# channable/alfred-margaret

Hardware: AMD Instinct MI355X
Metric: GiB/s haystack bytes scanned (match-emitting runLower, 100k-needle automaton) (higher is better)
Workload: dtype u8

## Files before the change

### alfred-margaret_amd/api.py

```python
import ctypes as C
import os

import numpy as np

from . import build as _build

CASE_SENSITIVE = 0
IGNORE_CASE = 1

AM_OK = 0
AM_ERR_INVALID, AM_ERR_NO_DEVICE, AM_ERR_HIP, AM_ERR_OOM, AM_ERR_UNSUPPORTED = -1, -2, -3, -4, -5


class AmError(RuntimeError):
    def __init__(self, code, msg):
        super().__init__("libam error %d: %s" % (code, msg))
        self.code = code


class _Match:
    __slots__ = ()

    def __repr__(self):
        return "am.MATCH"
# ... 1944 lines not shown
SF_MODES = ("count", "emit", "any", "ids")


def decode_sf_variant(word):
    word = int(word)
    if not word & 1:
        return None
    return {"ic": bool(word & 2), "mode": SF_MODES[(word >> 2) & 3], "ilp": (word >> 4) & 3, "lw": (word >> 16) & 255, "short": bool(word & 64), "dbg": bool(word & 128),
            "light": bool(word & 256), "children": bool(word & 512)}


def sf_last_variant():
    return decode_sf_variant(libam().am_debug_sf_last_variant())


def bounds_report():
    f, l, u = C.c_uint64(0), C.c_uint32(0), C.c_uint32(0)
    check(libam().am_debug_bounds_report(C.byref(f), C.byref(l), C.byref(u)))
    return int(f.value), int(l.value), int(u.value)


def image_version():
    return int(libam().am_image_version())


def lower_code_point(cp):
    return int(libam().am_lower_code_point(cp))


def unlower_code_point(cp):
# ... 49 lines not shown
```

### alfred-margaret_amd/csrc/am_abi.cpp

```cpp
#include "am_host.h"

#include <condition_variable>
#include <deque>
#include <sys/mman.h>

using namespace am;
using namespace am::dev;
using namespace am::host;

static_assert(sizeof(am_match) == sizeof(Record), "am_match must mirror the device record");
static_assert(offsetof(am_match, end_pos) == offsetof(Record, end_pos) && offsetof(am_match, haystack) == offsetof(Record, haystack) &&
                  offsetof(am_match, state) == offsetof(Record, state), "am_match layout");


static thread_local std::string g_err;
namespace am { int abi_fail(int code, const std::string& msg) { g_err = msg; return code; } }

namespace am {
namespace host {

Runtime g_rt;

int ensure_runtime()
{
// ... 208 lines not shown
{
    Orphans& o = orphans();
    std::lock_guard<std::mutex> lk(o.mu);
    for (int d = 0; d < kMaxDev; d++) {
        if (oneshot[d]) { o.batches[d].push_back(oneshot[d]); oneshot[d] = nullptr; }
        if (own[d]) { o.streams[d].push_back(own[d]); own[d] = nullptr; }
    }
    if (pin || pin_res) { o.pins.push_back(Orphans::Pins{pin, pin_cap, pin_res, pin_res_cap}); pin = pin_res = nullptr; }
    for (int k = 0; k < 2; k++) if (pin_ev[k] && pin_ev_dev >= 0) { o.events[pin_ev_dev].push_back(pin_ev[k]); pin_ev[k] = nullptr; }
}
}


uint64_t am::host::next_image_generation() { static std::atomic<uint64_t> g{0}; return g.fetch_add(1, std::memory_order_relaxed) + 1u; }

int am::host::prepare(const am_automaton* ca, int case_mode, const Flavor** out)
{
    if (!ca) return fail(AM_ERR_INVALID, "null automaton");
    if (case_mode != AM_CASE_SENSITIVE && case_mode != AM_IGNORE_CASE) return fail(AM_ERR_INVALID, "bad case_mode");
    am_automaton* a = const_cast<am_automaton*>(ca);
    std::lock_guard<std::mutex> lk(a->mu);
    Flavor& f = a->fl[case_mode];
    if (!f.ready) {
        if (!a->has_ref) return fail(AM_ERR_UNSUPPORTED, "this handle was attached to an image of the other case mode");
        AM_TRY(ensure_runtime());
        ON_DEVICE(a->dev);
        std::vector<uint8_t> img; std::string err;
        if (case_mode == AM_CASE_SENSITIVE && !a->cs_image.empty()) img.swap(a->cs_image);
        else if (case_mode == AM_IGNORE_CASE && a->ic_pending.valid()) {
            am_automaton::Flat fl = a->ic_pending.get();
            if (fl.rc != 0) return fail(AM_ERR_INVALID, fl.err);
            img.swap(fl.img);
        }
        else {
            RefArrays ref{a->transitions.data(), a->transitions.size(), a->offsets.data(), a->offsets.size() - 1, a->root_ascii.data(), a->values_len.data()};
            if (flatten(ref, case_mode, img, err, a->lower.get()) != 0) return fail(AM_ERR_INVALID, err);
        }
        void* d = nullptr;
        hipError_t e = hipMalloc(&d, img.size());
        if (e != hipSuccess) return fail(AM_ERR_OOM, std::string("hipMalloc(image): ") + hipGetErrorString(e));
        e = hipMemcpy(d, img.data(), img.size(), hipMemcpyHostToDevice);
        if (e != hipSuccess) { (void)hipFree(d); return fail(AM_ERR_HIP, std::string("hipMemcpy(image): ") + hipGetErrorString(e)); }
        std::memcpy(&f.h, img.data(), sizeof(ImageHeader));
        f.d_image = d; f.bytes = img.size(); f.generation = next_image_generation(); f.ready = true;
    }
    *out = &f;
    return AM_OK;
}

extern "C" const char* am_last_error(void) { return g_err.c_str(); }

extern "C" int am_automaton_create_ex(const uint64_t* transitions, size_t n_transitions, const uint32_t* offsets, size_t n_states,
                                      const uint64_t* root_ascii, const uint32_t* values_len,
                                      const uint32_t* lower_from, const uint32_t* lower_to, size_t n_lower_pairs, am_automaton** out)
{
    if (!out) return fail(AM_ERR_INVALID, "out is null");
    *out = nullptr;
    if (!transitions || !offsets || !root_ascii || !values_len || n_states == 0) return fail(AM_ERR_INVALID, "null or empty automaton arrays");
    std::shared_ptr<const LowerTable> lower;
// ... 43 lines not shown
    return builtin_lower_table().hash;
}

extern "C" uint32_t am_lower_table_hash(const uint32_t* lower_from, const uint32_t* lower_to, size_t n_pairs)
{
    if (!lower_from || !lower_to) return builtin_lower_table().hash;
    LowerTable lt; std::string err;
    if (LowerTable::make(lower_from, lower_to, n_pairs, lt, err) != 0) { g_err = err; return 0; }
    return lt.hash;
}

extern "C" void am_automaton_destroy(am_automaton* a)
{
    if (!a) return;
    if (a->ic_pending.valid()) a->ic_pending.wait();
    for (Flavor& f : a->fl) if (f.d_image) (void)hipFree(f.d_image);
    delete a;
}

extern "C" int am_automaton_set_kernel(am_automaton* a, int k)
{
    if (!a || k < 0 || k > 3) return fail(AM_ERR_INVALID, "bad arguments");
    a->kernel_pref = k;
    return AM_OK;
}

extern "C" int am_automaton_image_size(const am_automaton* a, int case_mode, size_t* nbytes)
{
    const Flavor* f; AM_TRY(prepare(a, case_mode, &f));
    if (!nbytes) return fail(AM_ERR_INVALID, "nbytes is null");
    *nbytes = f->bytes;
// ... 12 lines not shown
extern "C" int am_automaton_from_image(const void* d_image, size_t nbytes, am_automaton** out)
{
    if (!out) return fail(AM_ERR_INVALID, "out is null");
    *out = nullptr;
    if (!d_image || nbytes < sizeof(ImageHeader)) return fail(AM_ERR_INVALID, "image too small");
    int dev = 0;
    AM_TRY(device_of_pointer(d_image, &dev));
    ON_DEVICE(dev);
    ImageHeader h;
    HIP_TRY(hipMemcpy(&h, d_image, sizeof(h), hipMemcpyDeviceToHost));
    if (!image_sections_in_bounds(h) || h.total_bytes > nbytes) return fail(AM_ERR_INVALID, "not an automaton image");
    void* d = nullptr;
    HIP_TRY(hipMalloc(&d, h.total_bytes));
    hipError_t e = hipMemcpy(d, d_image, h.total_bytes, hipMemcpyDeviceToDevice);
    if (e != hipSuccess) { (void)hipFree(d); return fail(AM_ERR_HIP, hipGetErrorString(e)); }
    am_automaton* a = new am_automaton();
    a->dev = dev;
    Flavor& f = a->fl[h.case_mode];
    f.h = h; f.d_image = d; f.bytes = h.total_bytes; f.generation = next_image_generation(); f.ready = true;
    *out = a;
    return AM_OK;
}

extern "C" int am_automaton_image_read(const am_automaton* a, int case_mode, void* host_dst, size_t nbytes)
{
    const Flavor* f; AM_TRY(prepare(a, case_mode, &f));
    if (!host_dst || nbytes < f->bytes) return fail(AM_ERR_INVALID, "destination too small");
    ON_DEVICE(a->dev);
    HIP_TRY(hipMemcpy(host_dst, f->d_image, f->bytes, hipMemcpyDeviceToHost));
    return AM_OK;
}

extern "C" int am_automaton_from_host_image(const void* image, size_t nbytes, am_automaton** out)
{
    if (!out) return fail(AM_ERR_INVALID, "out is null");
// ... 6 lines not shown
    if (((uintptr_t)image & 63u) != 0) {
        try { aligned_copy.resize(((size_t)h.total_bytes + 7) / 8 + 8); } catch (const std::exception&) { return fail(AM_ERR_OOM, "no memory for an aligned copy of the image"); }
        uint8_t* base = (uint8_t*)aligned_copy.data();
        base += (64 - ((uintptr_t)base & 63u)) & 63u;
        std::memcpy(base, image, (size_t)h.total_bytes);
        image = base;
    }
    if (image_checksum((const uint8_t*)image + sizeof(h), (size_t)h.total_bytes - sizeof(h)) != h.checksum) return fail(AM_ERR_INVALID, "automaton image is corrupt (checksum)");
    { std::string why; if (!image_body_valid((const uint8_t*)image, h, why)) return fail(AM_ERR_INVALID, why); }
    int dev = 0;
    AM_TRY(current_device(&dev));
    void* d = nullptr;
    HIP_TRY(hipMalloc(&d, h.total_bytes));
    hipError_t e = hipMemcpy(d, image, h.total_bytes, hipMemcpyHostToDevice);
    if (e != hipSuccess) { (void)hipFree(d); return fail(AM_ERR_HIP, hipGetErrorString(e)); }
    am_automaton* a = new am_automaton();
    a->dev = dev;
    Flavor& f = a->fl[h.case_mode];
    f.h = h; f.d_image = d; f.bytes = h.total_bytes; f.generation = next_image_generation(); f.ready = true;
    *out = a;
    return AM_OK;
}


int am::host::finish_batch(am_batch* b)
{
    b->hidx_ready = false;
    b->route_image = 0;
    if (b->total > 0) AM_TRY(b->hidx.ensure(((b->total >> kHidxShift) + 2) * sizeof(uint32_t)));
    AM_TRY(b->small.ensure(64));
    return AM_OK;
}

int am::host::upload_batch(const am_slice* hay, size_t n_hay, am_batch* b, bool oneshot)
{
// ... 828 lines not shown
```

### alfred-margaret_amd/csrc/am_device.h

```cpp
#pragma once
#include <hip/hip_runtime.h>

#include "am_image.h"
#include "am_subst_tpl.h"

namespace am {
namespace dev {

constexpr int kModeCount = 0;
constexpr int kModeEmit = 1;
constexpr int kModeAny = 2;
constexpr int kModeIds = 3;

struct alignas(16) Record { uint64_t end_pos; uint32_t haystack; uint32_t state; };

struct ScanOut {
    uint32_t* unit_counts;
    const uint64_t* unit_offsets;
    Record* records;
    Record* pool;
    uint32_t* block_next;
    uint32_t* pool_ctrl;
    uint32_t* unit_first;
    uint32_t* unit_slots;
// ... 14 lines not shown
constexpr uint32_t kSfBlockGrant = 32;
inline uint64_t pool_grant_slack(int n_cu, uint64_t n_units, bool two_per_cu)
{
    uint64_t w = (uint64_t)n_cu * (two_per_cu ? 32u : 16u);
    const uint64_t need = (n_units + 15u) / 16u * 16u;
    if (w > need) w = need;
    return w * kSfBlockGrant;
}

hipError_t launch_hidx(const BatchView& b, uint32_t* hidx, uint64_t n_entries, hipStream_t st, uint32_t* z0 = nullptr, uint64_t n0 = 0, uint32_t* z1 = nullptr, uint64_t n1 = 0);
uint64_t sf_chunks(const BatchView& b);
uint32_t sf_unit_chunks(const BatchView& b, int n_cu);
hipError_t launch_permute(const ScanOut& o, const uint64_t* unit_offsets, Record* out, uint64_t n_units, hipStream_t st);
uint64_t ac_units(const AcView& a, const BatchView& b);
size_t sf_lds_bytes(const SfView& s);
hipError_t launch_sf(bool ic, int mode, const SfView& s, const BatchView& b, const ScanOut& o, int n_cu, hipStream_t st);
uint32_t take_sf_last_variant();
hipError_t launch_ac(bool ic, int mode, const AcView& a, const BatchView& b, const ScanOut& o, hipStream_t st);
uint64_t dfa_units(const DfaView& d, const BatchView& b);
bool dfa_usable(const DfaView& d);
struct DfaLaunch {
    int n_cu; uint32_t workgroups, per_cu;
    uint32_t lds_rows, hot_rows, lds_n1, lds_n2;
    uint32_t walk; bool place_wide;
};
DfaLaunch dfa_launch_shape(const DfaView& d, const BatchView& b, int n_cu);
hipError_t launch_dfa(int mode, const DfaView& d, const BatchView& b, const ScanOut& o, const DfaLaunch& s, hipStream_t st);
hipError_t launch_dfa_sample(const DfaView& d, const uint8_t* text, uint64_t total, uint32_t n_samples, uint32_t len, uint32_t* out, hipStream_t st);
bool dfa_tokens_ok(const DfaView& d);
uint64_t dfa_token_superblocks(uint64_t records, uint32_t n_waves , uint64_t n_units);
uint64_t dfa_superblock_bytes();
// ... 205 lines not shown
```

### alfred-margaret_amd/csrc/am_flatten.cpp

```cpp
#include "am_flatten.h"

#include "am_config.h"

#include <algorithm>
#include <chrono>
#include <future>
#include <system_error>
#include <cstdio>
#include <cstdlib>
#include <cstring>
#include <string>
#include <unordered_map>
#include <vector>

namespace am {


namespace {
struct LowerPair { uint32_t from, to; };
const LowerPair kLower[] = {
#include "unicode_lower_tbl.inc"
};
constexpr size_t kNLower = sizeof(kLower) / sizeof(kLower[0]);
}
// ... 1264 lines not shown
    }
    if (h.dfa_n_states) {
        if (h.dfa_log2_classes < 3 || h.dfa_log2_classes > 8 || h.dfa_n_states >= kDfaStateMask || h.dfa_chunk < 64 || (h.dfa_chunk & 15u) || h.dfa_warm == 0 || h.root_vlen != 0) return false;
        if (h.dfa_n_rows == 0 || h.dfa_n_rows > h.dfa_n_states || h.dfa_n_rows >= (1u << 24) || h.dfa_n_single > h.dfa_n_states - h.dfa_n_rows) return false;
        good = good && ok(h.off_dfa_chain2, h.dfa_n_states - h.dfa_n_rows - h.dfa_n_single, 16) && (h.off_dfa_chain2 & 15u) == 0;
        if ((1u << h.dfa_hot_log2) > (1u << h.dfa_log2_classes) - 1u || h.dfa_hot_log2 > 8) return false;
        good = good && ok(h.off_dfa_hot, (uint64_t)h.dfa_n_rows << h.dfa_hot_log2, 4) && (h.off_dfa_hot & 15u) == 0;
        good = good && ok(h.off_dfa_next, (uint64_t)h.dfa_n_rows << h.dfa_log2_classes, 4) && ok(h.off_dfa_chain, (uint64_t)h.dfa_n_single + 1u, 8) && (h.off_dfa_chain & 7u) == 0 &&
               ok(h.off_dfa_out, h.dfa_n_states, 8) && ok(h.off_dfa_cls, 256, 1) &&
               (h.off_dfa_next & 15u) == 0 && (h.off_dfa_out & 7u) == 0 && ok(h.off_dfa_fail, h.dfa_n_states, 4) && h.dfa_rare_log2_cap >= 4 && h.dfa_rare_log2_cap <= 30 &&
               ok(h.off_dfa_rare, 1ull << h.dfa_rare_log2_cap, 16) && (h.off_dfa_rare & 15u) == 0;
    }
    return good;
}

}
```

### alfred-margaret_amd/csrc/am_flatten.h

```cpp
#pragma once
#include <stddef.h>
#include <stdint.h>

#include <string>
#include <unordered_map>
#include <vector>

#include "am_image.h"

namespace am {

struct RefArrays {
    const uint64_t* transitions; size_t n_transitions;
    const uint32_t* offsets;
    size_t n_states;
    const uint64_t* root_ascii;
    const uint32_t* values_len;
};

struct LowerTable {
    std::vector<uint32_t> from, to;
    std::unordered_multimap<uint32_t, uint32_t> inverse;
    uint32_t hash = 0;
    static int make(const uint32_t* from, const uint32_t* to, size_t n, LowerTable& out, std::string& err);
    uint32_t lower(uint32_t cp) const;
    void unlower(uint32_t cp, std::vector<uint32_t>& out) const;
};
const LowerTable& builtin_lower_table();

int flatten(const RefArrays& ref, int case_mode, std::vector<uint8_t>& image, std::string& err, const LowerTable* lower_table = nullptr);

uint64_t image_checksum(const uint8_t* p, size_t n);
bool image_sections_in_bounds(const ImageHeader& h);
bool image_body_valid(const uint8_t* image, const ImageHeader& h, std::string& err);

uint32_t simple_lower(uint32_t cp);
void unlower(uint32_t cp, std::vector<uint32_t>& out);

}
```

### alfred-margaret_amd/csrc/am_host.h

```cpp
#pragma once
#include "../../include/am.h"
#include "../../include/am_debug.h"

#include <hip/hip_runtime.h>

#include <algorithm>
#include <atomic>
#include <chrono>
#include <cstdio>
#include <cstdlib>
#include <cstring>
#include <functional>
#include <future>
#include <map>
#include <memory>
#include <mutex>
#include <string>
#include <thread>
#include <vector>

#include "am_config.h"
#include "am_device.h"
#include "am_flatten.h"

// ... 83 lines not shown
        return AM_OK;
    }
    void release()
    {
        if (p) { (void)hipFree(p); g_device_buffer_bytes.fetch_sub(cap, std::memory_order_relaxed); }
        p = nullptr; cap = 0;
    }
};

struct Flavor {
    bool ready = false;
    void* d_image = nullptr;
    size_t bytes = 0;
    uint64_t generation = 0;
    ImageHeader h;
};
uint64_t next_image_generation();

}
}

struct am_automaton {
    int dev = 0;
    std::vector<uint64_t> transitions, root_ascii;
    std::vector<uint32_t> offsets, values_len;
    bool has_ref = false;
    std::shared_ptr<const am::LowerTable> lower;
    std::vector<uint8_t> cs_image;
    struct Flat { int rc = 0; std::string err; std::vector<uint8_t> img; };
    std::future<Flat> ic_pending;
    int kernel_pref = 0;
    std::mutex mu;
// ... 141 lines not shown
```

### alfred-margaret_amd/csrc/am_image.h

```cpp
#pragma once
#include <stdint.h>
#include <stddef.h>

#if defined(__HIPCC__)
#include <hip/hip_runtime.h>
#define AM_HD __host__ __device__ __forceinline__
#else
#define AM_HD inline
#endif

namespace am {

constexpr uint32_t kImageMagic = 0x31474D41u;
constexpr uint32_t kImageVersion = 19;
constexpr uint32_t kUnicodeLowerVersion = 0x0E00;
constexpr uint32_t kNone = 0xFFFFFFFFu;
constexpr uint64_t kWildcard = 0x200000ull;
constexpr uint32_t kHidxShift = 10;
constexpr uint32_t kSfChunk = 1024;

struct ImageHeader {
    uint32_t magic, version, case_mode, flags;
    uint64_t total_bytes;
    uint32_t n_states, max_needle_cps, root_vlen, ac_chunk;
// ... 204 lines not shown
    const uint32_t up = __builtin_amdgcn_bitop3_b32(ge_a, gt_z, x, 0x10);
#else
    const uint32_t up = ge_a & ~gt_z & ~x;
#endif
    return x | ((up >> 2) & 0x20202020u);
}

constexpr uint32_t kBloomMul = 0x9E3779B1u;
constexpr uint32_t kBloomMaskLog2 = 9;
constexpr uint32_t kBloomMasks = 1u << kBloomMaskLog2;
AM_HD uint32_t bloom_key(uint32_t w, bool ignore_case) { return ignore_case ? w | kBloomCaseBits : w; }
AM_HD uint32_t bloom_tier_key(uint32_t key, uint32_t tier, bool ignore_case) { return ignore_case ? key | (kBloomCaseBits >> (8u * (4u - tier))) : key; }
AM_HD uint32_t bloom_hash(uint32_t key, uint32_t tier) { return (key + (4u - tier) * 0x7F4A7C15u) * kBloomMul; }
AM_HD uint32_t bloom_word(uint32_t h, uint32_t log2_words) { return h >> (32u - log2_words); }
AM_HD uint32_t bloom_mask_index(uint32_t h) { return (h >> 2) & (kBloomMasks - 1u); }
AM_HD uint32_t bloom_mask_entry(uint32_t i)
{
    uint32_t x = (i + 1u) * 0x9E3779B1u;
    x ^= x >> 15; x *= 0x85EBCA6Bu; x ^= x >> 13; x *= 0xC2B2AE35u; x ^= x >> 16;
    uint32_t m = 0;
    for (uint32_t k = 0; k < 4u; k++) {
        uint32_t b = (x >> (5u * k)) & 31u;
        while (m & (1u << b)) b = (b + 1u) & 31u;
        m |= 1u << b;
    }
    return m;
}
AM_HD uint32_t bloom_mask(uint32_t h, const uint32_t* tab = nullptr) { return tab ? tab[bloom_mask_index(h)] : bloom_mask_entry(bloom_mask_index(h)); }
AM_HD bool bloom_hit(uint32_t v, uint32_t h, const uint32_t* tab = nullptr) { const uint32_t m = bloom_mask(h, tab); return (v & m) == m; }
constexpr uint32_t kScanRotShift = 11;
AM_HD uint32_t rotr32(uint32_t m, uint32_t r) { return (m >> r) | (m << ((32u - r) & 31u)); }
AM_HD uint32_t scan_rot(uint32_t h) { return (h >> kScanRotShift) & 31u; }
AM_HD uint32_t scan_mask(uint32_t h, const uint32_t* tab = nullptr) { return rotr32(bloom_mask(h, tab), scan_rot(h)); }
AM_HD bool scan_hit(uint32_t v, uint32_t h, const uint32_t* tab = nullptr) { const uint32_t m = scan_mask(h, tab); return (v & m) == m; }

AM_HD uint32_t tier_slot(uint32_t key, uint32_t log2_cap) { return (key * 0x85EBCA6Bu) >> (32u - log2_cap); }

AM_HD uint32_t tier_lookup(const u32x2* tab, uint32_t log2_cap, uint32_t key)
{
    const uint32_t cap_mask = (1u << log2_cap) - 1u;
    uint32_t i = tier_slot(key, log2_cap);
    for (;;) {
        u32x2 e = tab[i];
        if (e.y == kNone) return kNone;
        if (e.x == key) return e.y;
        i = (i + 1u) & cap_mask;
    }
}

// ... 683 lines not shown
```

### alfred-margaret_amd/csrc/am_kernels.hip

```cpp
#include <hip/hip_runtime.h>

#include <atomic>
#include <cstdlib>
#include <type_traits>

#include "am_bounds.h"
#include "am_config.h"
#include "am_device.h"
#include "am_wave.h"

AM_BOUNDS_TU("am_kernels.hip")

namespace am {
namespace dev {


__global__ void k_hidx(const uint64_t* __restrict__ offsets, uint32_t n_hay, uint64_t total, uint32_t* __restrict__ hidx, uint64_t n_entries,
                       uint32_t* __restrict__ z0, uint64_t n0, uint32_t* __restrict__ z1, uint64_t n1)
{
    const uint64_t k = (uint64_t)blockIdx.x * blockDim.x + threadIdx.x;
    const uint64_t stride = (uint64_t)gridDim.x * blockDim.x;
    for (uint64_t i = k; i < n0; i += stride) z0[i] = 0u;
    for (uint64_t i = k; i < n1; i += stride) z1[i] = 0u;
    if (k >= n_entries) return;
// ... 8 lines not shown
}


constexpr int kSfThreads = 1024;
constexpr int kSfWaves = kSfThreads / 64;
constexpr int kSfLightThreads = 256;
constexpr uint64_t kSfLightChunks = 16;
constexpr int kSfQ1 = 128;
constexpr int kSfQ2 = 256;
constexpr uint32_t kSfMaxUnitChunks = 64;
constexpr uint32_t kSfWqIters = 2;
constexpr uint32_t kSfEpochChunks = 16;
constexpr int kSfStage = 1056;
constexpr uint32_t kSfMaskBytes = kBloomMasks * 4u;

template <bool IC, int MODE, int ILP, int LW, bool SHORT, bool DBG, int NT = kSfThreads, bool CHILDREN = false>
__global__ __launch_bounds__(NT) void k_sf(SfView s, BatchView b, ScanOut o, uint64_t n_chunks)
{
    constexpr int kSfThreads = NT, kSfWaves = NT / 64;
    constexpr bool kFlagMode = MODE == kModeAny || MODE == kModeIds;
    constexpr bool CH = CHILDREN, children = CHILDREN;
    constexpr uint32_t kEpoch = kFlagMode ? 4u : CH ? 8u : kSfEpochChunks;
    extern __shared__ __attribute__((aligned(16))) uint32_t lds[];
    const uint32_t words = 1u << s.bloom_log2_words;
    uint32_t* masks = lds;
    uint32_t* bloom = lds + kBloomMasks;
    uint8_t* stage_all = reinterpret_cast<uint8_t*>(bloom + words);
    uint16_t* q1_all = reinterpret_cast<uint16_t*>(stage_all + kSfWaves * kSfStage);
    uint16_t* q2_all = q1_all + kSfWaves * kSfQ1;

    for (uint32_t i = threadIdx.x; i < kBloomMasks; i += kSfThreads) masks[i] = bloom_mask_entry(i);
    for (uint32_t i = threadIdx.x; i < words; i += kSfThreads) bloom[i] = s.scan_bloom[i];
    __syncthreads();

    const uint32_t lane = threadIdx.x & 63u, wave = __builtin_amdgcn_readfirstlane(threadIdx.x >> 6);
    const uint32_t stage = kSfMaskBytes + 4u * words + wave * (uint32_t)kSfStage;
    const uint32_t q1 = kSfMaskBytes + 4u * words + (uint32_t)kSfWaves * kSfStage + wave * (uint32_t)(kSfQ1 * 2);
    const uint32_t q2 = kSfMaskBytes + 4u * words + (uint32_t)kSfWaves * (kSfStage + kSfQ1 * 2) + wave * (uint32_t)(kSfQ2 * 2);
    const uint32_t wq_cap = o.wq_cap;
    const uint32_t wq = kSfMaskBytes + 4u * words + (uint32_t)kSfWaves * (kSfStage + kSfQ1 * 2 + kSfQ2 * 2) + wave * (wq_cap * 64u);
    uint32_t wq_n = 0;
    (void)stage_all; (void)q1_all; (void)q2_all;
    const uint64_t n_waves = (uint64_t)gridDim.x * kSfWaves;
    const uint32_t log2_words = s.bloom_log2_words, tiers = s.tiers & ~kSfKeyFold;
    const uint32_t UC = o.unit_chunks;
    const uint64_t n_units = (n_chunks + UC - 1) / UC;
// ... 437 lines not shown
            if (!last_of_unit) {
                next_c3 = (uint32_t)__builtin_amdgcn_readlane((int)d3, 63);
                next_c4 = (uint32_t)__builtin_amdgcn_readlane((int)d4, 63);
            }
            __builtin_amdgcn_s_setprio(0);
            uint32_t cand = 0;
            if (!kFlagMode || !skip) {
                uint32_t h[16], v[16], m[16];
                const uint32_t sh_word = 32u - log2_words;
#pragma unroll
                for (int k = 0; k < 16; k++) {
                    const int j = k >> 2, sh = k & 3;
                    const uint32_t w = sh == 3 ? f[j + 1] : __builtin_amdgcn_alignbyte(f[j + 1], f[j], sh + 1);
                    h[k] = w * kBloomMul;
                }
#pragma unroll
                for (int k = 15; k >= 0; k--) {
                    if (LW) v[k] = lds_read_u32(kSfMaskBytes + ((h[k] >> (30 - LW)) & (((1u << LW) - 1u) << 2)));
                    else v[k] = lds_read_u32(kSfMaskBytes + ((h[k] >> sh_word) << 2));
                    m[k] = lds_read_u32(h[k] & ((kBloomMasks - 1u) << 2));
                }
                __builtin_amdgcn_sched_barrier(0);
#pragma unroll
                for (int k = 15; k >= 0; k--) {
                    const uint32_t mr = rotr32(m[k], scan_rot(h[k]));
                    cand = shift_in_eq(cand, v[k] & mr, mr);
                }
            }
            if (SHORT && (!kFlagMode || !skip)) {
#pragma unroll
                for (int k = 0; k < 16; k++) {
                    const int j = k >> 2, sh = k & 3;
                    const uint32_t w = sh == 3 ? f[j + 1] : __builtin_amdgcn_alignbyte(f[j + 1], f[j], sh + 1);
                    if (sf_filter_short<true>(bloom, log2_words, tiers, w, masks)) cand |= 1u << k;
                }
            }
            __builtin_amdgcn_s_setprio(2);
            if (ci == tail_ci)
            if (p0 + 16 > b.total) cand &= p0 < b.total ? (1u << (uint32_t)(b.total - p0)) - 1u : 0u;
            if (timing) { asm volatile("" :: "v"(cand)); tick(t_filter); }

// ... 179 lines not shown
}
uint64_t ac_units(const AcView& a, const BatchView& b) { return (b.total + a.chunk - 1) / a.chunk; }

static size_t sf_lds_bytes_w(const SfView& s, int waves) { return kSfMaskBytes + ((size_t)4 << s.bloom_log2_words) + (size_t)waves * (kSfStage + kSfQ1 * sizeof(uint16_t) + kSfQ2 * sizeof(uint16_t)); }
static uint32_t sf_wq_cap(const SfView& s, int waves)
{
    const size_t base = sf_lds_bytes_w(s, waves), limit = 160 * 1024;
    if (base >= limit) return 0;
    size_t cap = (limit - base) / ((size_t)waves * 64);
    if (cap > 128) cap = 128;
    return cap >= 64 ? (uint32_t)cap : 0u;
}
size_t sf_lds_bytes(const SfView& s) { return sf_lds_bytes_w(s, kSfWaves); }

constexpr uint32_t kSfVariantValid = 1u, kSfVariantIc = 2u, kSfVariantModeShift = 2, kSfVariantIlpShift = 4, kSfVariantShort = 1u << 6, kSfVariantDbg = 1u << 7,
                   kSfVariantLight = 1u << 8, kSfVariantChildren = 1u << 9, kSfVariantLwShift = 16;
static std::atomic<uint32_t> g_sf_last_variant{0};
uint32_t take_sf_last_variant() { return g_sf_last_variant.exchange(0, std::memory_order_relaxed); }

template <bool IC, int MODE, int ILP, int LW, bool SHORT, bool DBG = false, int NT = kSfThreads, bool CHILDREN = false>
static hipError_t launch_sf_v(const SfView& s, const BatchView& b, const ScanOut& o, int n_cu, hipStream_t st)
{
    constexpr int waves_per_wg = NT / 64;
    constexpr bool kFlagMode = MODE == kModeAny || MODE == kModeIds;
    const uint32_t wq_cap = kFlagMode ? 0u : sf_wq_cap(s, waves_per_wg);
    const size_t lds = sf_lds_bytes_w(s, waves_per_wg) + (size_t)waves_per_wg * wq_cap * 64;
    static bool attr_set = false;
    if (!attr_set) {
        if (hipFuncSetAttribute(reinterpret_cast<const void*>(&k_sf<IC, MODE, ILP, LW, SHORT, DBG, NT, CHILDREN>), hipFuncAttributeMaxDynamicSharedMemorySize, 160 * 1024) != hipSuccess)
            (void)hipGetLastError();
        attr_set = true;
    }
    const uint64_t n_chunks = sf_chunks(b);
    const int per_cu = NT == kSfThreads ? (lds <= 80 * 1024 ? 2 : 1) : 8;
    uint64_t blocks = (uint64_t)n_cu * per_cu;
    const uint64_t n_units = (n_chunks + o.unit_chunks - 1) / o.unit_chunks;
    const uint64_t need = (n_units + waves_per_wg - 1) / waves_per_wg;
    if (blocks > need) blocks = need;
    if (blocks == 0) return hipSuccess;
    g_sf_last_variant.store(kSfVariantValid | (IC ? kSfVariantIc : 0u) | ((uint32_t)MODE << kSfVariantModeShift) | ((uint32_t)ILP << kSfVariantIlpShift) | (SHORT ? kSfVariantShort : 0u) |
                            (DBG ? kSfVariantDbg : 0u) | (NT == kSfLightThreads ? kSfVariantLight : 0u) | (CHILDREN ? kSfVariantChildren : 0u) | ((uint32_t)LW << kSfVariantLwShift),
                            std::memory_order_relaxed);
    ScanOut oo = o;
    oo.wq_cap = wq_cap;
    oo.wq_iters = kSfWqIters;
    if (n_units <= blocks * waves_per_wg) oo.next_unit = nullptr;
    hipLaunchKernelGGL((k_sf<IC, MODE, ILP, LW, SHORT, DBG, NT, CHILDREN>), dim3((uint32_t)blocks), dim3(NT), lds, st, s, b, oo, n_chunks);
    return hipGetLastError();
}

static uint64_t* g_sf_dbg = nullptr;
hipError_t read_sf_wave_records(uint64_t* out, size_t n_waves)
{
    if (!g_sf_dbg) return hipErrorInvalidValue;
    if (n_waves == 0) { hipError_t e = hipMemcpy(out, g_sf_dbg + 16 + 2 * 8192, 64, hipMemcpyDeviceToHost); if (e == hipSuccess) e = hipMemset(g_sf_dbg + 16 + 2 * 8192, 0, 64); return e; }
    return hipMemcpy(out, g_sf_dbg + 16, 16 * (n_waves < 8192 ? n_waves : 8192), hipMemcpyDeviceToHost);
}

hipError_t read_sf_phase_cycles(uint64_t* out5)
{
    for (int i = 0; i < 16; i++) out5[i] = 0;
    if (!g_sf_dbg) return hipSuccess;
    hipError_t e = hipMemcpy(out5, g_sf_dbg, 128, hipMemcpyDeviceToHost);
    if (e == hipSuccess) e = hipMemset(g_sf_dbg, 0, 128);
    return e;
}

template <bool IC, int MODE>
static hipError_t launch_sf_t(const SfView& s, const BatchView& b, const ScanOut& o, int n_cu, hipStream_t st)
{
    const bool lw15 = s.bloom_log2_words == 15;
    constexpr bool kFlagMode = MODE == kModeAny || MODE == kModeIds;
    if constexpr (MODE == kModeIds) {
        if (sf_chunks(b) <= kSfLightChunks)
            return (s.tiers & 7u) ? launch_sf_v<IC, MODE, 2, 0, true, false, kSfLightThreads>(s, b, o, n_cu, st) : launch_sf_v<IC, MODE, 2, 0, false, false, kSfLightThreads>(s, b, o, n_cu, st);
        return (s.tiers & 7u) ? launch_sf_v<IC, MODE, 2, 0, true>(s, b, o, n_cu, st) : launch_sf_v<IC, MODE, 2, 0, false>(s, b, o, n_cu, st);
    } else {
    if (o.dbg && !kFlagMode) {
        if (!lw15) return launch_sf_v<IC, MODE, 2, 0, true, true>(s, b, o, n_cu, st);
        return (s.tiers & 7u) ? launch_sf_v<IC, MODE, 2, 15, true, true>(s, b, o, n_cu, st) : launch_sf_v<IC, MODE, 2, 15, false, true>(s, b, o, n_cu, st);
    }
    if (sf_chunks(b) <= kSfLightChunks)
        return (s.tiers & 7u) ? launch_sf_v<IC, MODE, 2, 0, true, false, kSfLightThreads>(s, b, o, n_cu, st) : launch_sf_v<IC, MODE, 2, 0, false, false, kSfLightThreads>(s, b, o, n_cu, st);
    if (!lw15 && s.t4_children && !(s.tiers & 7u) && !kFlagMode) return launch_sf_v<IC, MODE, 2, 0, false, false, kSfThreads, true>(s, b, o, n_cu, st);
    const bool few = s.tier_log2_cap[3] <= 15u;
    if (s.tiers & 7u) {
        if (few) return lw15 ? launch_sf_v<IC, MODE, 1, 15, true>(s, b, o, n_cu, st) : launch_sf_v<IC, MODE, 1, 0, true>(s, b, o, n_cu, st);
        return lw15 ? launch_sf_v<IC, MODE, 2, 15, true>(s, b, o, n_cu, st) : launch_sf_v<IC, MODE, 2, 0, true>(s, b, o, n_cu, st);
    }
    if (few) return lw15 ? launch_sf_v<IC, MODE, 1, 15, false>(s, b, o, n_cu, st) : launch_sf_v<IC, MODE, 1, 0, false>(s, b, o, n_cu, st);
    return lw15 ? launch_sf_v<IC, MODE, 2, 15, false>(s, b, o, n_cu, st) : launch_sf_v<IC, MODE, 2, 0, false>(s, b, o, n_cu, st);
    }
}

hipError_t launch_sf(bool ic, int mode, const SfView& s, const BatchView& b, const ScanOut& o_in, int n_cu, hipStream_t st)
{
    ScanOut o = o_in;
    o.two_always = 0;
    static uint64_t* dbg = nullptr;
    if (cfg::on(cfg::kSfTrace)) {
        if (!dbg) { if (hipMalloc((void**)&dbg, 256 + 16 * 8192) != hipSuccess) dbg = nullptr; else (void)hipMemset(dbg, 0, 256 + 16 * 8192); }
        o.dbg = dbg;
        g_sf_dbg = dbg;
    }
    if (ic) {
        if (mode == kModeCount) return launch_sf_t<true, kModeCount>(s, b, o, n_cu, st);
        if (mode == kModeEmit) return launch_sf_t<true, kModeEmit>(s, b, o, n_cu, st);
        if (mode == kModeIds) return launch_sf_t<true, kModeIds>(s, b, o, n_cu, st);
        return launch_sf_t<true, kModeAny>(s, b, o, n_cu, st);
    }
    if (mode == kModeCount) return launch_sf_t<false, kModeCount>(s, b, o, n_cu, st);
    if (mode == kModeEmit) return launch_sf_t<false, kModeEmit>(s, b, o, n_cu, st);
    if (mode == kModeIds) return launch_sf_t<false, kModeIds>(s, b, o, n_cu, st);
    return launch_sf_t<false, kModeAny>(s, b, o, n_cu, st);
}

}
}
```

### alfred-margaret_amd/csrc/am_run.cpp

```cpp
#include "am_host.h"

using namespace am;
using namespace am::dev;
using namespace am::host;

namespace {

using AcLauncher = hipError_t (*)(bool ic, int mode, const AcView& a, const BatchView& b, const ScanOut& o, hipStream_t st);
std::atomic<AcLauncher> g_ac_launcher{nullptr};

constexpr uint64_t kDfaMinBytes = 32ull << 20;
constexpr uint64_t kDfaSampleBytes = 32ull << 20;
constexpr uint32_t kDfaEndsPerKiB = 48;

struct Plan {
    const Flavor* f; bool ic; bool use_sf; bool nothing; uint64_t n_units; uint32_t unit_chunks; int n_cu;
    bool use_dfa;
    DfaView dfa;
    DfaLaunch dfa_shape{};
    bool dense;
    AcView ac; SfView sf; BatchView bv;
    am_batch* batch;
    uint32_t* next_unit;
};
// ... 61 lines not shown
    if (p.use_sf) { if (!b->small.p) return fail(AM_ERR_INVALID, "batch without its counter block (not made by am_batch_upload / am_batch_from_device)"); p.next_unit = (uint32_t*)b->small.p + 8; }
    p.n_cu = g_rt.dev[b->dev].n_cu;
    p.batch = b;
    p.n_units = p.nothing ? 0 : (p.use_sf ? (sf_chunks(p.bv) + p.unit_chunks - 1) / p.unit_chunks : p.use_dfa ? dfa_units(p.dfa, p.bv) : ac_units(p.ac, p.bv));
    if (p.n_units >= 0x7FFFFFF0ull) return fail(AM_ERR_UNSUPPORTED, "batch too large for one launch; split it");
    if (p.use_dfa && !p.nothing) { ON_DEVICE(b->dev); p.dfa_shape = dfa_launch_shape(p.dfa, p.bv, p.n_cu); }
    return AM_OK;
}

int launch_scan_kernel(const Plan& p, int mode, const ScanOut& o, hipStream_t st)
{
    if (p.use_sf) {
        ScanOut os = o;
        os.next_unit = p.next_unit;
        Prof pr("sf", st);
        HIP_TRY(launch_sf(p.ic, mode, p.sf, p.bv, os, p.n_cu, st));
    }
    else if (p.use_dfa) {
        Prof pr("dfa", st);
        HIP_TRY(launch_dfa(mode, p.dfa, p.bv, o, p.dfa_shape, st));
    }
    else {
        const AcLauncher ac = g_ac_launcher.load(std::memory_order_acquire);
        if (!ac) return fail(AM_ERR_UNSUPPORTED, "the general AC kernel is not loaded");
        Prof pr("ac", st);
        HIP_TRY(ac(p.ic, mode, p.ac, p.bv, o, st));
    }
    return AM_OK;
}

int build_hidx(const Plan& p, am_batch* b, hipStream_t st)
// ... 418 lines not shown
```

Before: 1121.

## Add two-word blocked Bloom prefilter for large tier-4-only automata in scan kernel

```diff
diff --git a/alfred-margaret_amd/api.py b/alfred-margaret_amd/api.py
--- a/alfred-margaret_amd/api.py
+++ b/alfred-margaret_amd/api.py
@@ -1982,6 +1982,14 @@
     return decode_sf_variant(libam().am_debug_sf_last_variant())
 
 
+SF_VARIANT_W2 = 1 << 10
+
+
+def sf_last_variant_w2():
+    word = int(libam().am_debug_sf_last_variant())
+    return decode_sf_variant(word), bool(word & SF_VARIANT_W2)
+
+
 def bounds_report():
     f, l, u = C.c_uint64(0), C.c_uint32(0), C.c_uint32(0)
     check(libam().am_debug_bounds_report(C.byref(f), C.byref(l), C.byref(u)))
diff --git a/alfred-margaret_amd/csrc/am_abi.cpp b/alfred-margaret_amd/csrc/am_abi.cpp
--- a/alfred-margaret_amd/csrc/am_abi.cpp
+++ b/alfred-margaret_amd/csrc/am_abi.cpp
@@ -246,6 +246,26 @@
 
 uint64_t am::host::next_image_generation() { static std::atomic<uint64_t> g{0}; return g.fetch_add(1, std::memory_order_relaxed) + 1u; }
 
+int am::host::attach_scan2(Flavor& f, const void* host_image)
+{
+    if (!scan2_wanted(f.h)) return AM_OK;
+    std::vector<uint32_t> words;
+    if (host_image) scan2_derive(f.h, (const uint8_t*)host_image + f.h.off_t4_slots, words);
+    else {
+        std::vector<SfSlot> slots((size_t)2 << f.h.tier_log2_cap[3]);
+        HIP_TRY(hipMemcpy(slots.data(), (const uint8_t*)f.d_image + f.h.off_t4_slots, slots.size() * sizeof(SfSlot), hipMemcpyDeviceToHost));
+        scan2_derive(f.h, slots.data(), words);
+    }
+    if (words.empty()) return AM_OK;
+    void* d = nullptr;
+    hipError_t e = hipMalloc(&d, words.size() * 4);
+    if (e != hipSuccess) return fail(AM_ERR_OOM, std::string("hipMalloc(two-word filter): ") + hipGetErrorString(e));
+    e = hipMemcpy(d, words.data(), words.size() * 4, hipMemcpyHostToDevice);
+    if (e != hipSuccess) { (void)hipFree(d); return fail(AM_ERR_HIP, std::string("hipMemcpy(two-word filter): ") + hipGetErrorString(e)); }
+    f.d_scan2 = d;
+    return AM_OK;
+}
+
 int am::host::prepare(const am_automaton* ca, int case_mode, const Flavor** out)
 {
     if (!ca) return fail(AM_ERR_INVALID, "null automaton");
@@ -274,7 +294,9 @@
         e = hipMemcpy(d, img.data(), img.size(), hipMemcpyHostToDevice);
         if (e != hipSuccess) { (void)hipFree(d); return fail(AM_ERR_HIP, std::string("hipMemcpy(image): ") + hipGetErrorString(e)); }
         std::memcpy(&f.h, img.data(), sizeof(ImageHeader));
-        f.d_image = d; f.bytes = img.size(); f.generation = next_image_generation(); f.ready = true;
+        f.d_image = d;
+        if (int rc = attach_scan2(f, img.data())) { (void)hipFree(d); f.d_image = nullptr; return rc; }
+        f.bytes = img.size(); f.generation = next_image_generation(); f.ready = true;
     }
     *out = &f;
     return AM_OK;
@@ -348,7 +370,7 @@
 {
     if (!a) return;
     if (a->ic_pending.valid()) a->ic_pending.wait();
-    for (Flavor& f : a->fl) if (f.d_image) (void)hipFree(f.d_image);
+    for (Flavor& f : a->fl) { if (f.d_image) (void)hipFree(f.d_image); if (f.d_scan2) (void)hipFree(f.d_scan2); }
     delete a;
 }
 
@@ -391,11 +413,13 @@
     HIP_TRY(hipMalloc(&d, h.total_bytes));
     hipError_t e = hipMemcpy(d, d_image, h.total_bytes, hipMemcpyDeviceToDevice);
     if (e != hipSuccess) { (void)hipFree(d); return fail(AM_ERR_HIP, hipGetErrorString(e)); }
-    am_automaton* a = new am_automaton();
+    std::unique_ptr<am_automaton> a(new am_automaton());
     a->dev = dev;
     Flavor& f = a->fl[h.case_mode];
-    f.h = h; f.d_image = d; f.bytes = h.total_bytes; f.generation = next_image_generation(); f.ready = true;
-    *out = a;
+    f.h = h; f.d_image = d;
+    if (int rc = attach_scan2(f, nullptr)) { (void)hipFree(d); return rc; }
+    f.bytes = h.total_bytes; f.generation = next_image_generation(); f.ready = true;
+    *out = a.release();
     return AM_OK;
 }
 
@@ -432,11 +456,13 @@
     HIP_TRY(hipMalloc(&d, h.total_bytes));
     hipError_t e = hipMemcpy(d, image, h.total_bytes, hipMemcpyHostToDevice);
     if (e != hipSuccess) { (void)hipFree(d); return fail(AM_ERR_HIP, hipGetErrorString(e)); }
-    am_automaton* a = new am_automaton();
+    std::unique_ptr<am_automaton> a(new am_automaton());
     a->dev = dev;
     Flavor& f = a->fl[h.case_mode];
-    f.h = h; f.d_image = d; f.bytes = h.total_bytes; f.generation = next_image_generation(); f.ready = true;
-    *out = a;
+    f.h = h; f.d_image = d;
+    if (int rc = attach_scan2(f, image)) { (void)hipFree(d); return rc; }
+    f.bytes = h.total_bytes; f.generation = next_image_generation(); f.ready = true;
+    *out = a.release();
     return AM_OK;
 }
 
diff --git a/alfred-margaret_amd/csrc/am_device.h b/alfred-margaret_amd/csrc/am_device.h
--- a/alfred-margaret_amd/csrc/am_device.h
+++ b/alfred-margaret_amd/csrc/am_device.h
@@ -52,7 +52,7 @@
 hipError_t launch_permute(const ScanOut& o, const uint64_t* unit_offsets, Record* out, uint64_t n_units, hipStream_t st);
 uint64_t ac_units(const AcView& a, const BatchView& b);
 size_t sf_lds_bytes(const SfView& s);
-hipError_t launch_sf(bool ic, int mode, const SfView& s, const BatchView& b, const ScanOut& o, int n_cu, hipStream_t st);
+hipError_t launch_sf(bool ic, int mode, const SfView& s, const BatchView& b, const ScanOut& o, int n_cu, hipStream_t st, const uint32_t* scan2 = nullptr);
 uint32_t take_sf_last_variant();
 hipError_t launch_ac(bool ic, int mode, const AcView& a, const BatchView& b, const ScanOut& o, hipStream_t st);
 uint64_t dfa_units(const DfaView& d, const BatchView& b);
diff --git a/alfred-margaret_amd/csrc/am_flatten.cpp b/alfred-margaret_amd/csrc/am_flatten.cpp
--- a/alfred-margaret_amd/csrc/am_flatten.cpp
+++ b/alfred-margaret_amd/csrc/am_flatten.cpp
@@ -1302,4 +1302,46 @@
     return good;
 }
 
-}
+bool scan2_wanted(const ImageHeader& h)
+{
+    return h.sf_enabled && h.sf_bloom_log2_words == kScan2Log2Words && (h.sf_tiers & 7u) == 0u && (h.sf_tiers & 8u) != 0u;
+}
+
+void scan2_derive(const ImageHeader& h, const void* slots, std::vector<uint32_t>& words)
+{
+    words.clear();
+    if (!scan2_wanted(h)) return;
+    const bool ic = h.case_mode == 1;
+    const size_t n_slots = (size_t)2 << h.tier_log2_cap[3];
+    std::vector<uint32_t> keys;
+    for (size_t i = 0; i < n_slots; i++) {
+        uint32_t kf[2];
+        std::memcpy(kf, (const uint8_t*)slots + i * sizeof(SfSlot) + offsetof(SfSlot, key), sizeof(kf));
+        if (kf[1] & kSlotOccupied) keys.push_back(bloom_key(kf[0], ic));
+    }
+    std::sort(keys.begin(), keys.end());
+    keys.erase(std::unique(keys.begin(), keys.end()), keys.end());
+    if (keys.size() <= kScan2MinKeys) return;
+    words.assign((size_t)1 << kScan2Log2Words, 0u);
+    for (const uint32_t key : keys) {
+        const uint32_t hh = bloom_hash(key, 4), m = scan2_mask(hh);
+        words[bloom_word(hh, kScan2Log2Words)] |= m; words[scan2_word2(hh)] |= m;
+    }
+}
+
+}
+
+extern "C" long long amflat_scan2_filter(const void* image, size_t nbytes, uint32_t* out, size_t cap_words)
+{
+    using namespace am;
+    ImageHeader h;
+    if (!image || nbytes < sizeof(h)) return -1;
+    std::memcpy(&h, image, sizeof(h));
+    if (!image_sections_in_bounds(h) || h.total_bytes > nbytes) return -1;
+    std::vector<uint32_t> words;
+    scan2_derive(h, (const uint8_t*)image + h.off_t4_slots, words);
+    if (words.empty()) return 0;
+    if (!out || cap_words < words.size()) return -1;
+    std::memcpy(out, words.data(), words.size() * 4);
+    return (long long)words.size();
+}
diff --git a/alfred-margaret_amd/csrc/am_flatten.h b/alfred-margaret_amd/csrc/am_flatten.h
--- a/alfred-margaret_amd/csrc/am_flatten.h
+++ b/alfred-margaret_amd/csrc/am_flatten.h
@@ -34,6 +34,9 @@
 bool image_sections_in_bounds(const ImageHeader& h);
 bool image_body_valid(const uint8_t* image, const ImageHeader& h, std::string& err);
 
+bool scan2_wanted(const ImageHeader& h);
+void scan2_derive(const ImageHeader& h, const void* slots, std::vector<uint32_t>& words);
+
 uint32_t simple_lower(uint32_t cp);
 void unlower(uint32_t cp, std::vector<uint32_t>& out);
 
diff --git a/alfred-margaret_amd/csrc/am_host.h b/alfred-margaret_amd/csrc/am_host.h
--- a/alfred-margaret_amd/csrc/am_host.h
+++ b/alfred-margaret_amd/csrc/am_host.h
@@ -121,8 +121,10 @@
     size_t bytes = 0;
     uint64_t generation = 0;
     ImageHeader h;
+    void* d_scan2 = nullptr;
 };
 uint64_t next_image_generation();
+int attach_scan2(Flavor& f, const void* host_image);
 
 }
 }
diff --git a/alfred-margaret_amd/csrc/am_image.h b/alfred-margaret_amd/csrc/am_image.h
--- a/alfred-margaret_amd/csrc/am_image.h
+++ b/alfred-margaret_amd/csrc/am_image.h
@@ -242,12 +242,12 @@
 AM_HD uint32_t bloom_hash(uint32_t key, uint32_t tier) { return (key + (4u - tier) * 0x7F4A7C15u) * kBloomMul; }
 AM_HD uint32_t bloom_word(uint32_t h, uint32_t log2_words) { return h >> (32u - log2_words); }
 AM_HD uint32_t bloom_mask_index(uint32_t h) { return (h >> 2) & (kBloomMasks - 1u); }
-AM_HD uint32_t bloom_mask_entry(uint32_t i)
+AM_HD uint32_t bloom_mask_entry(uint32_t i, uint32_t nbits = 4u)
 {
     uint32_t x = (i + 1u) * 0x9E3779B1u;
     x ^= x >> 15; x *= 0x85EBCA6Bu; x ^= x >> 13; x *= 0xC2B2AE35u; x ^= x >> 16;
     uint32_t m = 0;
-    for (uint32_t k = 0; k < 4u; k++) {
+    for (uint32_t k = 0; k < nbits; k++) {
         uint32_t b = (x >> (5u * k)) & 31u;
         while (m & (1u << b)) b = (b + 1u) & 31u;
         m |= 1u << b;
@@ -261,6 +261,12 @@
 AM_HD uint32_t scan_rot(uint32_t h) { return (h >> kScanRotShift) & 31u; }
 AM_HD uint32_t scan_mask(uint32_t h, const uint32_t* tab = nullptr) { return rotr32(bloom_mask(h, tab), scan_rot(h)); }
 AM_HD bool scan_hit(uint32_t v, uint32_t h, const uint32_t* tab = nullptr) { const uint32_t m = scan_mask(h, tab); return (v & m) == m; }
+constexpr uint32_t kScan2Bits = 3u;
+constexpr uint32_t kScan2Log2Words = 15u;
+constexpr uint32_t kScan2MinKeys = 3u << kScan2Log2Words;
+AM_HD uint32_t scan2_word2(uint32_t h) { return (h >> (32u - kScan2Log2Words)) ^ ((h >> 2) & ((1u << kScan2Log2Words) - 1u)); }
+AM_HD uint32_t scan2_mask(uint32_t h) { return rotr32(bloom_mask_entry(bloom_mask_index(h), kScan2Bits), scan_rot(h)); }
+AM_HD bool scan2_hit(const uint32_t* f, uint32_t h) { const uint32_t m = scan2_mask(h); return (f[bloom_word(h, kScan2Log2Words)] & f[scan2_word2(h)] & m) == m; }
 
 AM_HD uint32_t tier_slot(uint32_t key, uint32_t log2_cap) { return (key * 0x85EBCA6Bu) >> (32u - log2_cap); }
 
diff --git a/alfred-margaret_amd/csrc/am_kernels.hip b/alfred-margaret_amd/csrc/am_kernels.hip
--- a/alfred-margaret_amd/csrc/am_kernels.hip
+++ b/alfred-margaret_amd/csrc/am_kernels.hip
@@ -46,7 +46,8 @@
 constexpr int kSfStage = 1056;
 constexpr uint32_t kSfMaskBytes = kBloomMasks * 4u;
 
-template <bool IC, int MODE, int ILP, int LW, bool SHORT, bool DBG, int NT = kSfThreads, bool CHILDREN = false>
+constexpr int kSfW2Group = 8;
+template <bool IC, int MODE, int ILP, int LW, bool SHORT, bool DBG, int NT = kSfThreads, bool CHILDREN = false, bool W2 = false>
 __global__ __launch_bounds__(NT) void k_sf(SfView s, BatchView b, ScanOut o, uint64_t n_chunks)
 {
     constexpr int kSfThreads = NT, kSfWaves = NT / 64;
@@ -61,7 +62,8 @@
     uint16_t* q1_all = reinterpret_cast<uint16_t*>(stage_all + kSfWaves * kSfStage);
     uint16_t* q2_all = q1_all + kSfWaves * kSfQ1;
 
-    for (uint32_t i = threadIdx.x; i < kBloomMasks; i += kSfThreads) masks[i] = bloom_mask_entry(i);
+    static_assert(!W2 || (LW == (int)kScan2Log2Words && !SHORT && !CHILDREN), "the two-word filter is for 2^15 words without tier probes");
+    for (uint32_t i = threadIdx.x; i < kBloomMasks; i += kSfThreads) masks[i] = W2 ? bloom_mask_entry(i, kScan2Bits) : bloom_mask_entry(i);
     for (uint32_t i = threadIdx.x; i < words; i += kSfThreads) bloom[i] = s.scan_bloom[i];
     __syncthreads();
 
@@ -529,17 +531,39 @@
                     const uint32_t w = sh == 3 ? f[j + 1] : __builtin_amdgcn_alignbyte(f[j + 1], f[j], sh + 1);
                     h[k] = w * kBloomMul;
                 }
-#pragma unroll
-                for (int k = 15; k >= 0; k--) {
-                    if (LW) v[k] = lds_read_u32(kSfMaskBytes + ((h[k] >> (30 - LW)) & (((1u << LW) - 1u) << 2)));
-                    else v[k] = lds_read_u32(kSfMaskBytes + ((h[k] >> sh_word) << 2));
-                    m[k] = lds_read_u32(h[k] & ((kBloomMasks - 1u) << 2));
-                }
-                __builtin_amdgcn_sched_barrier(0);
-#pragma unroll
-                for (int k = 15; k >= 0; k--) {
-                    const uint32_t mr = rotr32(m[k], scan_rot(h[k]));
-                    cand = shift_in_eq(cand, v[k] & mr, mr);
+                if constexpr (W2) {
+                    constexpr uint32_t kWordBytes = ((1u << kScan2Log2Words) - 1u) << 2;
+                    uint32_t v2[16];
+#pragma unroll
+                    for (int g = 16 - kSfW2Group; g >= 0; g -= kSfW2Group) {
+#pragma unroll
+                        for (int k = g + kSfW2Group - 1; k >= g; k--) {
+                            const uint32_t a1 = (h[k] >> (30 - LW)) & kWordBytes;
+                            v[k] = lds_read_u32(kSfMaskBytes + a1);
+                            v2[k] = lds_read_u32(kSfMaskBytes + (a1 ^ (h[k] & kWordBytes)));
+                            m[k] = lds_read_u32(h[k] & ((kBloomMasks - 1u) << 2));
+                        }
+                        __builtin_amdgcn_sched_barrier(0);
+#pragma unroll
+                        for (int k = g + kSfW2Group - 1; k >= g; k--) {
+                            const uint32_t mr = rotr32(m[k], scan_rot(h[k]));
+                            cand = shift_in_eq(cand, v[k] & v2[k] & mr, mr);
+                        }
+                        if (g) __builtin_amdgcn_sched_barrier(0);
+                    }
+                } else {
+#pragma unroll
+                    for (int k = 15; k >= 0; k--) {
+                        if (LW) v[k] = lds_read_u32(kSfMaskBytes + ((h[k] >> (30 - LW)) & (((1u << LW) - 1u) << 2)));
+                        else v[k] = lds_read_u32(kSfMaskBytes + ((h[k] >> sh_word) << 2));
+                        m[k] = lds_read_u32(h[k] & ((kBloomMasks - 1u) << 2));
+                    }
+                    __builtin_amdgcn_sched_barrier(0);
+#pragma unroll
+                    for (int k = 15; k >= 0; k--) {
+                        const uint32_t mr = rotr32(m[k], scan_rot(h[k]));
+                        cand = shift_in_eq(cand, v[k] & mr, mr);
+                    }
                 }
             }
             if (SHORT && (!kFlagMode || !skip)) {
@@ -749,11 +773,11 @@
 size_t sf_lds_bytes(const SfView& s) { return sf_lds_bytes_w(s, kSfWaves); }
 
 constexpr uint32_t kSfVariantValid = 1u, kSfVariantIc = 2u, kSfVariantModeShift = 2, kSfVariantIlpShift = 4, kSfVariantShort = 1u << 6, kSfVariantDbg = 1u << 7,
-                   kSfVariantLight = 1u << 8, kSfVariantChildren = 1u << 9, kSfVariantLwShift = 16;
+                   kSfVariantLight = 1u << 8, kSfVariantChildren = 1u << 9, kSfVariantW2 = 1u << 10, kSfVariantLwShift = 16;
 static std::atomic<uint32_t> g_sf_last_variant{0};
 uint32_t take_sf_last_variant() { return g_sf_last_variant.exchange(0, std::memory_order_relaxed); }
 
-template <bool IC, int MODE, int ILP, int LW, bool SHORT, bool DBG = false, int NT = kSfThreads, bool CHILDREN = false>
+template <bool IC, int MODE, int ILP, int LW, bool SHORT, bool DBG = false, int NT = kSfThreads, bool CHILDREN = false, bool W2 = false>
 static hipError_t launch_sf_v(const SfView& s, const BatchView& b, const ScanOut& o, int n_cu, hipStream_t st)
 {
     constexpr int waves_per_wg = NT / 64;
@@ -762,7 +786,7 @@
     const size_t lds = sf_lds_bytes_w(s, waves_per_wg) + (size_t)waves_per_wg * wq_cap * 64;
     static bool attr_set = false;
     if (!attr_set) {
-        if (hipFuncSetAttribute(reinterpret_cast<const void*>(&k_sf<IC, MODE, ILP, LW, SHORT, DBG, NT, CHILDREN>), hipFuncAttributeMaxDynamicSharedMemorySize, 160 * 1024) != hipSuccess)
+        if (hipFuncSetAttribute(reinterpret_cast<const void*>(&k_sf<IC, MODE, ILP, LW, SHORT, DBG, NT, CHILDREN, W2>), hipFuncAttributeMaxDynamicSharedMemorySize, 160 * 1024) != hipSuccess)
             (void)hipGetLastError();
         attr_set = true;
     }
@@ -774,13 +798,13 @@
     if (blocks > need) blocks = need;
     if (blocks == 0) return hipSuccess;
     g_sf_last_variant.store(kSfVariantValid | (IC ? kSfVariantIc : 0u) | ((uint32_t)MODE << kSfVariantModeShift) | ((uint32_t)ILP << kSfVariantIlpShift) | (SHORT ? kSfVariantShort : 0u) |
-                            (DBG ? kSfVariantDbg : 0u) | (NT == kSfLightThreads ? kSfVariantLight : 0u) | (CHILDREN ? kSfVariantChildren : 0u) | ((uint32_t)LW << kSfVariantLwShift),
+                            (DBG ? kSfVariantDbg : 0u) | (NT == kSfLightThreads ? kSfVariantLight : 0u) | (CHILDREN ? kSfVariantChildren : 0u) | (W2 ? kSfVariantW2 : 0u) | ((uint32_t)LW << kSfVariantLwShift),
                             std::memory_order_relaxed);
     ScanOut oo = o;
     oo.wq_cap = wq_cap;
     oo.wq_iters = kSfWqIters;
     if (n_units <= blocks * waves_per_wg) oo.next_unit = nullptr;
-    hipLaunchKernelGGL((k_sf<IC, MODE, ILP, LW, SHORT, DBG, NT, CHILDREN>), dim3((uint32_t)blocks), dim3(NT), lds, st, s, b, oo, n_chunks);
+    hipLaunchKernelGGL((k_sf<IC, MODE, ILP, LW, SHORT, DBG, NT, CHILDREN, W2>), dim3((uint32_t)blocks), dim3(NT), lds, st, s, b, oo, n_chunks);
     return hipGetLastError();
 }
 
@@ -801,8 +825,9 @@
     return e;
 }
 
+constexpr int kSfW2Ilp = 1;
 template <bool IC, int MODE>
-static hipError_t launch_sf_t(const SfView& s, const BatchView& b, const ScanOut& o, int n_cu, hipStream_t st)
+static hipError_t launch_sf_t(const SfView& s, const BatchView& b, const ScanOut& o, int n_cu, hipStream_t st, const uint32_t* scan2)
 {
     const bool lw15 = s.bloom_log2_words == 15;
     constexpr bool kFlagMode = MODE == kModeAny || MODE == kModeIds;
@@ -811,13 +836,18 @@
             return (s.tiers & 7u) ? launch_sf_v<IC, MODE, 2, 0, true, false, kSfLightThreads>(s, b, o, n_cu, st) : launch_sf_v<IC, MODE, 2, 0, false, false, kSfLightThreads>(s, b, o, n_cu, st);
         return (s.tiers & 7u) ? launch_sf_v<IC, MODE, 2, 0, true>(s, b, o, n_cu, st) : launch_sf_v<IC, MODE, 2, 0, false>(s, b, o, n_cu, st);
     } else {
+    const bool w2 = scan2 != nullptr && lw15 && !(s.tiers & 7u);
+    SfView s2 = s;
+    if (w2) s2.scan_bloom = scan2;
     if (o.dbg && !kFlagMode) {
+        if (w2 && sf_chunks(b) > kSfLightChunks) return launch_sf_v<IC, MODE, kSfW2Ilp, 15, false, true, kSfThreads, false, true>(s2, b, o, n_cu, st);
         if (!lw15) return launch_sf_v<IC, MODE, 2, 0, true, true>(s, b, o, n_cu, st);
         return (s.tiers & 7u) ? launch_sf_v<IC, MODE, 2, 15, true, true>(s, b, o, n_cu, st) : launch_sf_v<IC, MODE, 2, 15, false, true>(s, b, o, n_cu, st);
     }
     if (sf_chunks(b) <= kSfLightChunks)
         return (s.tiers & 7u) ? launch_sf_v<IC, MODE, 2, 0, true, false, kSfLightThreads>(s, b, o, n_cu, st) : launch_sf_v<IC, MODE, 2, 0, false, false, kSfLightThreads>(s, b, o, n_cu, st);
     if (!lw15 && s.t4_children && !(s.tiers & 7u) && !kFlagMode) return launch_sf_v<IC, MODE, 2, 0, false, false, kSfThreads, true>(s, b, o, n_cu, st);
+    if (w2) return launch_sf_v<IC, MODE, kSfW2Ilp, 15, false, false, kSfThreads, false, true>(s2, b, o, n_cu, st);
     const bool few = s.tier_log2_cap[3] <= 15u;
     if (s.tiers & 7u) {
         if (few) return lw15 ? launch_sf_v<IC, MODE, 1, 15, true>(s, b, o, n_cu, st) : launch_sf_v<IC, MODE, 1, 0, true>(s, b, o, n_cu, st);
@@ -828,7 +858,7 @@
     }
 }
 
-hipError_t launch_sf(bool ic, int mode, const SfView& s, const BatchView& b, const ScanOut& o_in, int n_cu, hipStream_t st)
+hipError_t launch_sf(bool ic, int mode, const SfView& s, const BatchView& b, const ScanOut& o_in, int n_cu, hipStream_t st, const uint32_t* scan2)
 {
     ScanOut o = o_in;
     o.two_always = 0;
@@ -839,16 +869,16 @@
         g_sf_dbg = dbg;
     }
     if (ic) {
-        if (mode == kModeCount) return launch_sf_t<true, kModeCount>(s, b, o, n_cu, st);
-        if (mode == kModeEmit) return launch_sf_t<true, kModeEmit>(s, b, o, n_cu, st);
-        if (mode == kModeIds) return launch_sf_t<true, kModeIds>(s, b, o, n_cu, st);
-        return launch_sf_t<true, kModeAny>(s, b, o, n_cu, st);
-    }
-    if (mode == kModeCount) return launch_sf_t<false, kModeCount>(s, b, o, n_cu, st);
-    if (mode == kModeEmit) return launch_sf_t<false, kModeEmit>(s, b, o, n_cu, st);
-    if (mode == kModeIds) return launch_sf_t<false, kModeIds>(s, b, o, n_cu, st);
-    return launch_sf_t<false, kModeAny>(s, b, o, n_cu, st);
-}
-
-}
-}
+        if (mode == kModeCount) return launch_sf_t<true, kModeCount>(s, b, o, n_cu, st, scan2);
+        if (mode == kModeEmit) return launch_sf_t<true, kModeEmit>(s, b, o, n_cu, st, scan2);
+        if (mode == kModeIds) return launch_sf_t<true, kModeIds>(s, b, o, n_cu, st, scan2);
+        return launch_sf_t<true, kModeAny>(s, b, o, n_cu, st, scan2);
+    }
+    if (mode == kModeCount) return launch_sf_t<false, kModeCount>(s, b, o, n_cu, st, scan2);
+    if (mode == kModeEmit) return launch_sf_t<false, kModeEmit>(s, b, o, n_cu, st, scan2);
+    if (mode == kModeIds) return launch_sf_t<false, kModeIds>(s, b, o, n_cu, st, scan2);
+    return launch_sf_t<false, kModeAny>(s, b, o, n_cu, st, scan2);
+}
+
+}
+}
diff --git a/alfred-margaret_amd/csrc/am_run.cpp b/alfred-margaret_amd/csrc/am_run.cpp
--- a/alfred-margaret_amd/csrc/am_run.cpp
+++ b/alfred-margaret_amd/csrc/am_run.cpp
@@ -99,7 +99,7 @@
         ScanOut os = o;
         os.next_unit = p.next_unit;
         Prof pr("sf", st);
-        HIP_TRY(launch_sf(p.ic, mode, p.sf, p.bv, os, p.n_cu, st));
+        HIP_TRY(launch_sf(p.ic, mode, p.sf, p.bv, os, p.n_cu, st, (const uint32_t*)p.f->d_scan2));
     }
     else if (p.use_dfa) {
         Prof pr("dfa", st);
```

Result: faster. 1180, median of 6 (+5.3%).
